# ufal/neuralmonkey

Hardware: NVIDIA H100
Metric: train_target_tokens_per_sec (higher is better)
Workload: dtype f32 storage; tensor-core products in fp16 (vocabulary) / tf32 with fp32 accumulation

## Files before the change

include/nmb200.h:

```cpp
#ifndef NMB200_H
#define NMB200_H

#include <stdint.h>

#ifdef __cplusplus
extern "C" {
#endif

#define NM_ABI_VERSION 1

#define NM_OK 0
#define NM_E_INVALID (-1)
#define NM_E_UNSUPPORTED (-2)
#define NM_E_NO_DEVICE (-3)

#define NM_ACT_NONE 0
#define NM_ACT_TANH 1
#define NM_ACT_RELU 2
#define NM_ACT_SIGMOID 3

#define NM_GEMM_AUTO 0
#define NM_GEMM_SIMT 1
#define NM_GEMM_TC 2

// ... 79 lines not shown
                float* lse, float* xent, int64_t* argmax, int64_t M, int64_t V,
                int64_t ldl, void* stream);
int nm_xent_bwd(const float* logits, const int64_t* targets, const float* weights,
                const float* lse, const float* scale, float* dlogits, int64_t M,
                int64_t V, int64_t ldl, void* stream);
int nm_log_softmax(const float* logits, const float* lse, float* logprobs,
                   int64_t M, int64_t V, int64_t ldl, void* stream);

int64_t nm_logits_xent_scratch(int64_t M, int64_t V);
int nm_logits_xent_fwd(const float* X, int64_t ldx, const float* W, int64_t ldw,
                       int transW, const float* b, int64_t unk_index, const int64_t* targets,
                       const float* weights, float* lse, float* xent,
                       int64_t* argmax, float* part, float* logits_out,
                       int64_t ldl, int64_t M, int64_t V, int64_t K, void* stream);
int nm_logits_xent_bwd(const float* X, int64_t ldx, const float* W, int64_t ldw,
                       int transW, const float* b, int64_t unk_index, const int64_t* targets,
                       const float* weights, const float* lse, const float* scale,
                       float* dlogits, int64_t ldd, int64_t M, int64_t V,
                       int64_t K, void* stream);

int nm_cast_f16(const float* src, int64_t ld_src, void* dst, int64_t ld_dst, int64_t rows,
                int64_t cols, const float* row_scale, int transpose, int extra_ones, void* stream);
int nm_gemm_f16(int64_t M, int64_t N, int64_t K, const void* A16, int64_t lda, const void* B16,
                int64_t ldb, float* C, int64_t ldc, const float* alpha_dev, const float* row_scale,
                float beta, int transposed, void* stream);
int nm_gemm_f16_tn(int64_t M, int64_t N, int64_t K, const void* A16, int64_t lda, const void* B16,
                   int64_t ldb, float* C, int64_t ldc, const float* alpha_dev, float beta, void* stream);
int nm_logits_xent_fwd16(const void* X16, int64_t ldx, const void* WT16, int64_t ldw, const float* b,
                         int64_t unk_index, const int64_t* targets, const float* weights, float* lse,
                         float* xent, int64_t* argmax, float* part, float* logits_out, int64_t ldl,
                         int64_t M, int64_t V, int64_t K, void* stream);
int nm_logits_xent_bwd16(const void* X16, int64_t ldx, const void* WT16, int64_t ldw, const float* b,
                         int64_t unk_index, const int64_t* targets, const float* mask, const float* lse,
                         void* dl16, int64_t ldd, void* dlT16, int64_t lddt, int64_t M, int64_t V,
                         int64_t K, void* stream);

int nm_beam_step(const float* logprobs, const float* logprob_sum,
                 const int32_t* lengths, const uint8_t* finished, float alpha,
                 float* scores, int64_t* word_ids, int32_t* beam_ids,
                 float* logprob_sum_out, int32_t* lengths_out,
                 uint8_t* finished_out, void* scratch, int64_t B, int64_t k,
                 int64_t V, void* stream);
int64_t nm_beam_scratch(int64_t B, int64_t k, int64_t V);
int nm_beam_gather(const void* x, const int32_t* beam_ids, void* out, int64_t B,
                   int64_t k, int64_t row_bytes, void* stream);

int nm_clip_adam_step(float* params, float* grads, float* m, float* v,
                      const int64_t* seg_off, const uint8_t* seg_reg, float* norms,
                      int64_t n, int64_t nseg, float grad_scale,
                      const float* grad_denominator, float lr_t,
                      float beta1, float beta2, float eps, float clip_norm,
                      float l1, float l2, float* l1l2_out,
                      const float* lr_t_dev ,
                      void* stream);

int nm_mha_fwd(const float* q, const float* k, const float* v,
               const float* key_mask, int causal, float* out, float* probs,
               int64_t B, int64_t Tq, int64_t Tk, int64_t heads, int64_t dh,
               void* stream);
int nm_mha_bwd(const float* q, const float* k, const float* v,
               const float* key_mask, int causal, const float* probs,
               const float* dout, float* dq, float* dk, float* dv,
               float* de_work , int64_t B,
               int64_t Tq, int64_t Tk, int64_t heads, int64_t dh, void* stream);
int nm_mha_fwd_drop(const float* q, const float* k, const float* v, const float* key_mask, int causal,
                    const float* drop_mask, float* out, float* probs, int64_t B, int64_t Tq,
                    int64_t Tk, int64_t heads, int64_t dh, void* stream);
int nm_mha_bwd_drop(const float* q, const float* k, const float* v, const float* key_mask, int causal,
// ... 73 lines not shown
```

neuralmonkey_b200/csrc/gemm_tc.cu:

```cuda
#include <cuda.h>
#include <cuda_fp16.h>
#include <stdlib.h>
#include <string.h>

#include "common.cuh"
#include "gemm_tc.h"
#include "tc_ptx.cuh"
#include "wgmma.cuh"

namespace nm {

constexpr int TC_BM = 128;
constexpr int TC_BK = 32;
constexpr int TC_THREADS = 384;
constexpr int TC_EPI_WARPS = 8;
constexpr int TC_A_BYTES = TC_BM * 128;
constexpr int TC_RING_BUDGET = 192 * 1024;

template <int BN>
struct TcCfg {
  static constexpr int B_BYTES = BN * 128;
  static constexpr int STAGE_BYTES = TC_A_BYTES + B_BYTES;
  static constexpr int STAGES = (TC_RING_BUDGET / STAGE_BYTES) > 4 ? 4 : (TC_RING_BUDGET / STAGE_BYTES);
  static constexpr int CT_PITCH = BN + 4;
  static constexpr int RING_BYTES = STAGES * STAGE_BYTES;
  static constexpr int CT_BYTES = TC_BM * CT_PITCH * 4;
  static constexpr int UNION_BYTES = RING_BYTES > CT_BYTES ? RING_BYTES : CT_BYTES;
  static constexpr int SMEM_BYTES = 1024  + UNION_BYTES + 256  +
                                    TC_EPI_WARPS * 4096 ;
  static_assert(SMEM_BYTES <= 227 * 1024, "more shared memory than an sm_90 block may have");
};
struct RowStats {
  float mx, sum, tgt;
  int32_t arg;
};

constexpr float TC_LOG2E = 1.4426950408889634f;

__device__ __forceinline__ float fast_ex2(float x) {
  float y;
  asm("ex2.approx.ftz.f32 %0, %1;" : "=f"(y) : "f"(x));
  return y;
}

__device__ __forceinline__ void load_bias32(const float* __restrict__ bias, int col0, int ncols,
                                            float (&b)[32]) {
  if (bias == nullptr) {
#pragma unroll
    for (int j = 0; j < 32; ++j) b[j] = 0.f;
    return;
  }
  if (ncols == 32 && ((reinterpret_cast<uintptr_t>(bias + col0) & 15) == 0)) {
#pragma unroll
    for (int j = 0; j < 32; j += 4) {
      const float4 v = __ldg(reinterpret_cast<const float4*>(bias + col0 + j));
      b[j] = v.x; b[j + 1] = v.y; b[j + 2] = v.z; b[j + 3] = v.w;
    }
  } else {
#pragma unroll
    for (int j = 0; j < 32; ++j) b[j] = (j < ncols) ? __ldg(bias + col0 + j) : 0.f;
  }
}

__device__ __forceinline__ void store32(float* __restrict__ c, const float (&x)[32], int ncols,
                                        bool vec_ok) {
  if (vec_ok && ncols == 32) {
#pragma unroll
    for (int j = 0; j < 32; j += 4)
      *reinterpret_cast<float4*>(c + j) = make_float4(x[j], x[j + 1], x[j + 2], x[j + 3]);
  } else {
#pragma unroll
    for (int j = 0; j < 32; ++j)
      if (j < ncols) c[j] = x[j];
  }
}

__device__ __forceinline__ void store32_coalesced(float* __restrict__ stage, float* __restrict__ C,
// ... 119 lines not shown
#pragma unroll
    for (int j = 0; j < 8; ++j) {
      float4 v = make_float4(x[4 * j], x[4 * j + 1], x[4 * j + 2], x[4 * j + 3]);
      if (add_bias && e.bias) {
        const float4 b = __ldg(reinterpret_cast<const float4*>(e.bias + col0 + 4 * j));
        v.x += b.x; v.y += b.y; v.z += b.z; v.w += b.w;
      }
      st4[lane * 8 + (j ^ (lane & 7))] = v;
    }
    __syncwarp();
    const int sub = lane >> 3, slot = lane & 7;
    const int64_t row_base = row - lane;
#pragma unroll
    for (int i = 0; i < 8; ++i) {
      const int r = 4 * i + sub;
      const float4 v = st4[r * 8 + (slot ^ (r & 7))];
      const int64_t grow = row_base + r;
      if (grow < M) red_add_v4(e.C + grow * e.ldc + col0 + 4 * slot, v);
    }
    __syncwarp();
    return;
  }
  if (row >= M) return;
  float* c = e.C + row * e.ldc + col0;
#pragma unroll
  for (int j = 0; j < 32; ++j)
    if (j < ncols) {
      float v = x[j];
      if (add_bias && e.bias) v += __ldg(e.bias + col0 + j);
      atomicAdd(c + j, v);
    }
}

template <typename T>
__device__ __forceinline__ void store32_transposed(T* __restrict__ ct, int64_t ldt, int64_t row, int col0,
                                                   int64_t M, int ncols, const float (&x)[32], float beta) {
  if (row >= M) return;
#pragma unroll
  for (int j = 0; j < 32; ++j) {
    if (j < ncols) {
      T* dst = ct + (int64_t)(col0 + j) * ldt + row;
      if constexpr (sizeof(T) == 2) {
        *dst = __float2half_rn(x[j]);
      } else {
        *dst = (beta != 0.f) ? (x[j] + *dst) : x[j];
      }
    }
  }
}

__device__ __forceinline__ void store32_half_coalesced(float* __restrict__ stage, __half* __restrict__ C,
                                                       int64_t ldc, int64_t row_base, int col0, int64_t M,
                                                       const float (&x)[32], int lane) {
  uint4* st4 = reinterpret_cast<uint4*>(stage);
#pragma unroll
  for (int j = 0; j < 4; ++j) {
    __half2 h0 = __floats2half2_rn(x[8 * j], x[8 * j + 1]), h1 = __floats2half2_rn(x[8 * j + 2], x[8 * j + 3]);
    __half2 h2 = __floats2half2_rn(x[8 * j + 4], x[8 * j + 5]), h3 = __floats2half2_rn(x[8 * j + 6], x[8 * j + 7]);
    uint4 v;
    v.x = *reinterpret_cast<uint32_t*>(&h0); v.y = *reinterpret_cast<uint32_t*>(&h1);
    v.z = *reinterpret_cast<uint32_t*>(&h2); v.w = *reinterpret_cast<uint32_t*>(&h3);
    st4[lane * 4 + (j ^ ((lane >> 1) & 3))] = v;
  }
  __syncwarp();
  const int sub = lane >> 2, slot = lane & 3;
#pragma unroll
  for (int i = 0; i < 4; ++i) {
    const int r = 8 * i + sub;
    const uint4 v = st4[r * 4 + (slot ^ ((r >> 1) & 3))];
    const int64_t grow = row_base + r;
    if (grow < M) *reinterpret_cast<uint4*>(C + grow * ldc + col0 + 8 * slot) = v;
  }
  __syncwarp();
}

__device__ __forceinline__ void epilogue_chunk_xent_bwd16(const TcEpilogue& e, const TcExt& ext, float (&x)[32],
                                                          int64_t row, int col0, int64_t M, int N, int target,
                                                          float row_lse2, float row_w,
                                                          float* __restrict__ stage, int lane) {
  if (col0 >= N) return;
  const int ncols = min(32, N - col0);
  float b[32];
  load_bias32(e.bias, col0, ncols, b);
#pragma unroll
  for (int j = 0; j < 32; ++j) x[j] += b[j];
  const int unk_rel = (int)e.unk_index - col0;
  if (unk_rel >= 0 && unk_rel < 32) {
#pragma unroll
    for (int j = 0; j < 32; ++j)
      if (j == unk_rel) x[j] += -1e9f;
  }
#pragma unroll
  for (int j = 0; j < 32; ++j) x[j] = fast_ex2(fmaf(x[j], TC_LOG2E, -row_lse2)) * row_w;
  const int t_rel = target - col0;
  if (t_rel >= 0 && t_rel < ncols) {
#pragma unroll
    for (int j = 0; j < 32; ++j)
      if (j == t_rel) x[j] -= row_w;
  }
  __half* c16 = reinterpret_cast<__half*>(ext.C16);
  const bool vec_ok = ncols == 32 && ((ext.ldc16 & 7) == 0) && ((reinterpret_cast<uintptr_t>(c16) & 15) == 0);
  if (vec_ok) {
    store32_half_coalesced(stage, c16, ext.ldc16, row - lane, col0, M, x, lane);
  } else if (row < M) {
#pragma unroll
    for (int j = 0; j < 32; ++j)
      if (j < ncols) c16[row * ext.ldc16 + col0 + j] = __float2half_rn(x[j]);
  }
  if (ext.C16T)
    store32_transposed(reinterpret_cast<__half*>(ext.C16T), ext.ldc16t, row, col0, M, ncols, x, 0.f);
}

__device__ __forceinline__ void epilogue_chunk_dense16(const TcEpilogue& e, const TcExt& ext, float (&x)[32],
                                                       int64_t row, int col0, int64_t M, int N, float factor,
                                                       bool vec_ok, float* __restrict__ stage, int lane,
                                                       RowStats& st) {
#pragma unroll
  for (int j = 0; j < 32; ++j) x[j] *= factor;
  if (!ext.transposed) {
    epilogue_chunk<TC_EPI_DENSE>(e, x, row, col0, M, N, st, -1, 0.f, 0.f, vec_ok, stage, lane);
    return;
  }
  if (col0 >= N) return;
  const int ncols = min(32, N - col0);
  if (e.bias) {
    float b[32];
    load_bias32(e.bias, col0, ncols, b);
#pragma unroll
    for (int j = 0; j < 32; ++j) x[j] += b[j];
  }
  store32_transposed(e.C, e.ldc, row, col0, M, ncols, x, e.beta);
}

__device__ __forceinline__ void load32_coalesced(float* __restrict__ stage, const float* __restrict__ src,
                                                 int64_t ld, int64_t row_base, int col0, int64_t M,
                                                 float (&x)[32], int lane) {
  float4* st4 = reinterpret_cast<float4*>(stage);
  const int sub = lane >> 3, slot = lane & 7;
#pragma unroll
  for (int i = 0; i < 8; ++i) {
    const int r = 4 * i + sub;
    const int64_t grow = row_base + r;
    float4 v = make_float4(0.f, 0.f, 0.f, 0.f);
// ... 352 lines not shown
typedef CUresult (*EncodeTiledFn)(CUtensorMap*, CUtensorMapDataType, cuuint32_t, void*,
                                  const cuuint64_t*, const cuuint64_t*, const cuuint32_t*,
                                  const cuuint32_t*, CUtensorMapInterleave, CUtensorMapSwizzle,
                                  CUtensorMapL2promotion, CUtensorMapFloatOOBfill);

static EncodeTiledFn get_encode_fn() {
  static EncodeTiledFn fn = nullptr;
  if (!fn) {
    void* p = nullptr;
    cudaDriverEntryPointQueryResult q;
    if (cudaGetDriverEntryPoint("cuTensorMapEncodeTiled", &p, cudaEnableDefault, &q) == cudaSuccess &&
        q == cudaDriverEntryPointSuccess)
      fn = reinterpret_cast<EncodeTiledFn>(p);
  }
  return fn;
}

static int make_map(CUtensorMap* map, const float* base, int64_t rows, int64_t cols, int64_t ld, uint32_t box_rows) {
  EncodeTiledFn fn = get_encode_fn();
  NM_REQUIRE(fn != nullptr, NM_E_NO_DEVICE, "tc_gemm: cuTensorMapEncodeTiled not available");
  const cuuint64_t gdim[2] = {(cuuint64_t)cols, (cuuint64_t)rows};
  const cuuint64_t gstride[1] = {(cuuint64_t)ld * 4};
  const cuuint32_t box[2] = {(cuuint32_t)TC_BK, box_rows};
  const cuuint32_t estr[2] = {1, 1};
  const CUresult r = fn(map, CU_TENSOR_MAP_DATA_TYPE_TFLOAT32, 2, const_cast<float*>(base), gdim, gstride, box, estr,
                        CU_TENSOR_MAP_INTERLEAVE_NONE, CU_TENSOR_MAP_SWIZZLE_128B,
                        CU_TENSOR_MAP_L2_PROMOTION_L2_128B, CU_TENSOR_MAP_FLOAT_OOB_FILL_NONE);
  NM_REQUIRE(r == CUDA_SUCCESS, NM_E_INVALID,
             "tc_gemm: cuTensorMapEncodeTiled failed (%d) rows=%lld cols=%lld ld=%lld", (int)r,
             (long long)rows, (long long)cols, (long long)ld);
  return NM_OK;
}

static int make_map16(CUtensorMap* map, const void* base, int64_t rows, int64_t cols, int64_t ld,
                      uint32_t box_rows) {
  EncodeTiledFn fn = get_encode_fn();
  NM_REQUIRE(fn != nullptr, NM_E_NO_DEVICE, "tc_gemm16: cuTensorMapEncodeTiled not available");
  const cuuint64_t gdim[2] = {(cuuint64_t)cols, (cuuint64_t)rows};
  const cuuint64_t gstride[1] = {(cuuint64_t)ld * 2};
  const cuuint32_t box[2] = {64, box_rows};
  const cuuint32_t estr[2] = {1, 1};
  const CUresult r = fn(map, CU_TENSOR_MAP_DATA_TYPE_FLOAT16, 2, const_cast<void*>(base), gdim, gstride, box,
                        estr, CU_TENSOR_MAP_INTERLEAVE_NONE, CU_TENSOR_MAP_SWIZZLE_128B,
                        CU_TENSOR_MAP_L2_PROMOTION_L2_128B, CU_TENSOR_MAP_FLOAT_OOB_FILL_NONE);
  NM_REQUIRE(r == CUDA_SUCCESS, NM_E_INVALID,
             "tc_gemm16: cuTensorMapEncodeTiled failed (%d) rows=%lld cols=%lld ld=%lld", (int)r,
             (long long)rows, (long long)cols, (long long)ld);
  return NM_OK;
}

static int make_operand(CUtensorMap* map, TcOperand* op, bool mn_major, const void* base, int64_t rows, int64_t cols,
                        int64_t ld, uint32_t box_rows, int esz) {
  memset(map, 0, sizeof(*map));
  *op = TcOperand{base, rows, cols, ld};
  if (mn_major) return NM_OK;
  if (esz == 4) return make_map(map, reinterpret_cast<const float*>(base), rows, cols, ld, box_rows);
  return make_map16(map, base, rows, cols, ld, box_rows);
}

bool tc_gemm_supported(int64_t M, int64_t N, int64_t K, int64_t lda, int64_t ldb, const void* A, const void* B) {
  if (M < 1 || N < 1 || K < 1) return false;
  if ((lda & 3) || (ldb & 3)) return false;
  if (A && (reinterpret_cast<uintptr_t>(A) & 15)) return false;
  if (B && (reinterpret_cast<uintptr_t>(B) & 15)) return false;
  if (M > 0x7fffffffLL || N > 0x7fffffffLL || K > 0x7fffffffLL) return false;
  return true;
}
// ... 233 lines not shown
```

neuralmonkey_b200/csrc/gemm_tc.h:

```cpp
#pragma once
#include <cuda_runtime.h>
#include <stdint.h>

namespace nm {

enum TcEpiMode {
  TC_EPI_DENSE = 0,
  TC_EPI_XENT_FWD = 1,
  TC_EPI_XENT_BWD = 2,
  TC_EPI_XENT_BWD16 = 3,
  TC_EPI_SOFTMAX = 4,
  TC_EPI_DSOFTMAX = 5,
};

constexpr int TC_XENT_BN = 256;

struct TcEpilogue {
  int mode;
  float* C;
  int64_t ldc;
  const float* bias;
  int act;
  float beta;
  int64_t unk_index;
  const int64_t* targets;
  const float* weights;
  const float* lse;
  const float* scale;
  float4* part;
};

struct TcExt {
  void* C16;
  int64_t ldc16;
  void* C16T;
  int64_t ldc16t;
  const float* alpha;
  const float* row_scale;
  int transposed;
};

struct TcBatch {
  int count, inner;
  int a_row_outer, a_row_inner, a_col_inner;
  int b_row_outer, b_row_inner, b_col_inner;
  int64_t c_outer, c_inner;
  float scale;
  int causal;
  const float* key_mask;
  const float* drop;
  float* C2;
  const float* P;
  int m_pad, n_pad;
};

int tc_gemm_batched_launch(int transA, int transB, int64_t M, int64_t N, int64_t K, const float* A, int64_t a_rows,
                           int64_t a_cols, int64_t lda, const float* B, int64_t b_rows, int64_t b_cols,
                           int64_t ldb, const TcEpilogue& epi, const TcBatch& bt, cudaStream_t s);

bool tc_gemm_supported(int64_t M, int64_t N, int64_t K, int64_t lda, int64_t ldb, const void* A, const void* B);

int tc_gemm_launch(int transA, int transB, int64_t M, int64_t N, int64_t K, const float* A,
                   int64_t lda, const float* B, int64_t ldb, const TcEpilogue& epi, cudaStream_t s);

int tc_gemm16_launch(int64_t M, int64_t N, int64_t K, const void* A, int64_t lda, const void* B,
                     int64_t ldb, const TcEpilogue& epi, const TcExt& ext, cudaStream_t s);

int tc_gemm16_mn_launch(int64_t M, int64_t N, int64_t K, const void* A, int64_t lda, const void* B,
                        int64_t ldb, const TcEpilogue& epi, const TcExt& ext, cudaStream_t s);

}
```

neuralmonkey_b200/csrc/tc_ptx.cuh:

```cuda
#pragma once
#include <cuda.h>
#include <cuda_fp16.h>
#include <cuda_runtime.h>
#include <stdint.h>

namespace nm {

__device__ __forceinline__ uint32_t smem_u32(const void* p) {
  return (uint32_t)__cvta_generic_to_shared(p);
}
__device__ __forceinline__ void mbar_init(uint32_t bar, uint32_t count) {
  asm volatile("mbarrier.init.shared::cta.b64 [%0], %1;" ::"r"(bar), "r"(count));
}
__device__ __forceinline__ void mbar_expect_tx(uint32_t bar, uint32_t bytes) {
  asm volatile("mbarrier.arrive.expect_tx.shared::cta.b64 _, [%0], %1;" ::"r"(bar), "r"(bytes)
               : "memory");
}
__device__ __forceinline__ void mbar_arrive(uint32_t bar) {
  asm volatile("mbarrier.arrive.shared::cta.b64 _, [%0];" ::"r"(bar) : "memory");
}
__device__ __forceinline__ void mbar_wait(uint32_t bar, uint32_t parity) {
  asm volatile(
      "{\n\t"
      ".reg .pred p;\n\t"
      "WAIT_LOOP:\n\t"
      "mbarrier.try_wait.parity.shared::cta.b64 p, [%0], %1;\n\t"
      "@p bra WAIT_DONE;\n\t"
      "bra WAIT_LOOP;\n\t"
      "WAIT_DONE:\n\t"
      "}" ::"r"(bar),
      "r"(parity)
      : "memory");
}
__device__ __forceinline__ void tma_load_2d(uint32_t dst, const CUtensorMap* map, uint32_t bar,
                                            int32_t c0, int32_t c1) {
  asm volatile(
      "cp.async.bulk.tensor.2d.shared::cluster.global.mbarrier::complete_tx::bytes"
      " [%0], [%1, {%3, %4}], [%2];" ::"r"(dst),
      "l"(reinterpret_cast<uint64_t>(map)), "r"(bar), "r"(c0), "r"(c1)
      : "memory");
}
__device__ __forceinline__ void mbar_expect_tx_only(uint32_t bar, uint32_t bytes) {
  asm volatile("mbarrier.expect_tx.relaxed.cta.shared::cta.b64 [%0], %1;" ::"r"(bar), "r"(bytes) : "memory");
}
__device__ __forceinline__ uint32_t to_tf32(float x) {
  uint32_t u;
  asm("cvt.rna.tf32.f32 %0, %1;" : "=r"(u) : "f"(x));
  return u;
}

__device__ __forceinline__ void wgmma_fence() { asm volatile("wgmma.fence.sync.aligned;" ::: "memory"); }
__device__ __forceinline__ void wgmma_commit() { asm volatile("wgmma.commit_group.sync.aligned;" ::: "memory"); }
template <int N>
__device__ __forceinline__ void wgmma_wait() {
  asm volatile("wgmma.wait_group.sync.aligned %0;" ::"n"(N) : "memory");
}
template <int R>
__device__ __forceinline__ void wgmma_fence_operands(float (&d)[R]) {
#pragma unroll
  for (int i = 0; i < R; ++i) asm volatile("" : "+f"(d[i])::"memory");
}

__device__ __forceinline__ uint64_t gmma_desc_sw128(uint32_t addr) {
  return (uint64_t)((addr & 0x3FFFFu) >> 4) | ((uint64_t)1 << 16) | ((uint64_t)(1024 >> 4) << 32) |
         ((uint64_t)1 << 62);
}

__device__ __forceinline__ uint64_t gmma_desc_sw128_mn(uint32_t addr) {
  return (uint64_t)((addr & 0x3FFFFu) >> 4) | ((uint64_t)(8192 >> 4) << 16) | ((uint64_t)(1024 >> 4) << 32) |
         ((uint64_t)1 << 62);
}

}
```

neuralmonkey_b200/csrc/xent16.cu:

```cuda
#include <cuda_fp16.h>

#include "common.cuh"
#include "gemm_tc.h"

namespace nm {

__global__ void cast_f16_kernel(const float* __restrict__ src, int64_t ld_src, __half* __restrict__ dst,
                                int64_t ld_dst, int64_t rows, int64_t cols,
                                const float* __restrict__ row_scale, int extra_ones) {
  const int64_t total = rows * ld_dst;
  for (int64_t i = blockIdx.x * (int64_t)blockDim.x + threadIdx.x; i < total;
       i += (int64_t)gridDim.x * blockDim.x) {
    const int64_t r = i / ld_dst, c = i - r * ld_dst;
    float v = 0.f;
    const float sc = row_scale ? row_scale[r] : 1.f;
    if (c < cols) v = src[r * ld_src + c] * sc;
    else if (c < cols + extra_ones) v = sc;
    dst[i] = __float2half_rn(v);
  }
}

__global__ void cast_transpose_f16_kernel(const float* __restrict__ src, int64_t ld_src,
                                          __half* __restrict__ dst, int64_t ld_dst, int64_t rows,
                                          int64_t cols, const float* __restrict__ row_scale,
                                          int extra_ones) {
  __shared__ float tile[32][33];
  const int64_t r0 = blockIdx.x * 32LL, c0 = blockIdx.y * 32LL;
  for (int i = threadIdx.y; i < 32; i += blockDim.y) {
    const int64_t r = r0 + i, c = c0 + threadIdx.x;
    float v = 0.f;
    if (r < rows) {
      const float sc = row_scale ? row_scale[r] : 1.f;
      if (c < cols) v = src[r * ld_src + c] * sc;
      else if (c < cols + extra_ones) v = sc;
    }
    tile[i][threadIdx.x] = v;
  }
  __syncthreads();
  for (int i = threadIdx.y; i < 32; i += blockDim.y) {
    const int64_t c = c0 + i, r = r0 + threadIdx.x;
    if (c < cols + extra_ones && r < ld_dst) dst[c * ld_dst + r] = __float2half_rn(tile[threadIdx.x][i]);
  }
}

}

using namespace nm;

extern "C" {

int nm_cast_f16(const float* src, int64_t ld_src, void* dst, int64_t ld_dst, int64_t rows, int64_t cols,
                const float* row_scale, int transpose, int extra_ones, void* stream) {
  NM_REQUIRE(src && dst && rows > 0 && cols > 0 && ld_src >= cols, NM_E_INVALID, "nm_cast_f16: bad arguments");
  cudaStream_t s = (cudaStream_t)stream;
  if (!transpose) {
    NM_REQUIRE(extra_ones >= 0 && ld_dst >= cols + extra_ones, NM_E_INVALID, "nm_cast_f16: bad destination pitch");
    const int64_t total = rows * ld_dst;
    const int64_t blocks = ceil_div(total, 256 * 4);
    const int64_t cap = (int64_t)sm_count() * 16;
    cast_f16_kernel<<<(unsigned)(blocks < cap ? blocks : cap), 256, 0, s>>>(
        src, ld_src, reinterpret_cast<__half*>(dst), ld_dst, rows, cols, row_scale, extra_ones);
  } else {
    NM_REQUIRE(ld_dst >= rows && extra_ones >= 0, NM_E_INVALID, "nm_cast_f16: bad destination pitch");
    const dim3 grid((unsigned)ceil_div(ld_dst, 32), (unsigned)ceil_div(cols + extra_ones, 32));
    cast_transpose_f16_kernel<<<grid, dim3(32, 8), 0, s>>>(src, ld_src, reinterpret_cast<__half*>(dst), ld_dst,
                                                          rows, cols, row_scale, extra_ones);
  }
  NM_LAUNCH_CHECK("nm_cast_f16");
  return NM_OK;
}

int nm_gemm_f16(int64_t M, int64_t N, int64_t K, const void* A16, int64_t lda, const void* B16, int64_t ldb,
                float* C, int64_t ldc, const float* alpha_dev, const float* row_scale, float beta,
                int transposed, void* stream) {
  NM_REQUIRE(A16 && B16 && C, NM_E_INVALID, "nm_gemm_f16: null pointer");
// ... 2 lines not shown
  TcEpilogue epi{};
  epi.mode = TC_EPI_DENSE;
  epi.C = C;
  epi.ldc = ldc;
  epi.act = NM_ACT_NONE;
  epi.beta = beta;
  epi.unk_index = -1;
  TcExt ext{};
  ext.alpha = alpha_dev;
  ext.row_scale = row_scale;
  ext.transposed = transposed;
  return tc_gemm16_launch(M, N, K, A16, lda, B16, ldb, epi, ext, (cudaStream_t)stream);
}

int nm_gemm_f16_tn(int64_t M, int64_t N, int64_t K, const void* A16, int64_t lda, const void* B16, int64_t ldb,
                   float* C, int64_t ldc, const float* alpha_dev, float beta, void* stream) {
  NM_REQUIRE(A16 && B16 && C, NM_E_INVALID, "nm_gemm_f16_tn: null pointer");
  NM_REQUIRE(beta == 0.f || beta == 1.f, NM_E_INVALID, "nm_gemm_f16_tn: beta must be 0 or 1");
  NM_REQUIRE(lda >= M && ldb >= N && ldc >= N, NM_E_INVALID, "nm_gemm_f16_tn: bad pitches");
  TcEpilogue epi{};
  epi.mode = TC_EPI_DENSE;
  epi.C = C;
  epi.ldc = ldc;
  epi.act = NM_ACT_NONE;
  epi.beta = beta;
  epi.unk_index = -1;
  TcExt ext{};
  ext.alpha = alpha_dev;
  return tc_gemm16_mn_launch(M, N, K, A16, lda, B16, ldb, epi, ext, (cudaStream_t)stream);
}

int nm_logits_xent_bwd16(const void* X16, int64_t ldx, const void* WT16, int64_t ldw, const float* b,
                         int64_t unk_index, const int64_t* targets, const float* mask, const float* lse,
                         void* dl16, int64_t ldd, void* dlT16, int64_t lddt, int64_t M, int64_t V, int64_t K,
                         void* stream) {
  NM_REQUIRE(X16 && WT16 && targets && lse && dl16, NM_E_INVALID, "nm_logits_xent_bwd16: null pointer");
  NM_REQUIRE(M > 0 && V > 0 && K > 0 && ldx >= K && ldw >= K && ldd >= V && (!dlT16 || lddt >= M),
             NM_E_INVALID, "nm_logits_xent_bwd16: bad sizes");
  TcEpilogue epi{};
  epi.mode = TC_EPI_XENT_BWD16;
  epi.bias = b;
  epi.unk_index = unk_index;
  epi.targets = targets;
  epi.weights = mask;
  epi.lse = lse;
  TcExt ext{};
  ext.C16 = dl16;
  ext.ldc16 = ldd;
  ext.C16T = dlT16;
  ext.ldc16t = lddt;
  return tc_gemm16_launch(M, V, K, X16, ldx, WT16, ldw, epi, ext, (cudaStream_t)stream);
}

}
```

neuralmonkey_b200/csrc/xent_tc.cu:

```cuda
#include "common.cuh"
#include "gemm_tc.h"

namespace nm {

__global__ void xent_combine_kernel(const float4* __restrict__ part, int64_t M, int64_t tiles_n,
                                    const int64_t* __restrict__ targets,
                                    const float* __restrict__ weights, float* __restrict__ lse,
                                    float* __restrict__ xent, int64_t* __restrict__ argmax) {
  const int lane = threadIdx.x & 31;
  const int64_t row = blockIdx.x * (int64_t)(blockDim.x >> 5) + (threadIdx.x >> 5);
  if (row >= M) return;
  float mx = -INFINITY, tgt = -INFINITY;
  int32_t arg = 0x7fffffff;
  for (int64_t t = lane; t < tiles_n; t += 32) {
    const float4 p = part[row * tiles_n + t];
    const int32_t a = __float_as_int(p.z);
    if (p.x > mx || (p.x == mx && a < arg)) { mx = p.x; arg = a; }
    tgt = fmaxf(tgt, p.w);
  }
#pragma unroll
  for (int o = 16; o > 0; o >>= 1) {
    const float omx = __shfl_xor_sync(0xffffffffu, mx, o);
    const int32_t oarg = __shfl_xor_sync(0xffffffffu, arg, o);
    if (omx > mx || (omx == mx && oarg < arg)) { mx = omx; arg = oarg; }
// ... 55 lines not shown
  return NM_OK;
}

int nm_logits_xent_bwd(const float* X, int64_t ldx, const float* W, int64_t ldw, int transW,
                       const float* b, int64_t unk_index, const int64_t* targets, const float* weights,
                       const float* lse, const float* scale, float* dlogits, int64_t ldd, int64_t M,
                       int64_t V, int64_t K, void* stream) {
  NM_REQUIRE(X && W && targets && lse && scale && dlogits, NM_E_INVALID,
             "nm_logits_xent_bwd: null pointer");
  NM_REQUIRE(M > 0 && V > 0 && K > 0 && ldx >= K && ldw >= (transW ? K : V) && ldd >= V, NM_E_INVALID,
             "nm_logits_xent_bwd: bad sizes");
  NM_REQUIRE(tc_gemm_supported(M, V, K, ldx, ldw, X, W), NM_E_UNSUPPORTED,
             "nm_logits_xent_bwd: operands not TMA-addressable (use nm_gemm + nm_xent_bwd)");
  TcEpilogue epi{};
  epi.mode = TC_EPI_XENT_BWD;
  epi.C = dlogits;
  epi.ldc = ldd;
  epi.bias = b;
  epi.unk_index = unk_index;
  epi.targets = targets;
  epi.weights = weights;
  epi.lse = lse;
  epi.scale = scale;
  return tc_gemm_launch(0, transW, M, V, K, X, ldx, W, ldw, epi, (cudaStream_t)stream);
}

int nm_logits_xent_fwd16(const void* X16, int64_t ldx, const void* WT16, int64_t ldw, const float* b,
                         int64_t unk_index, const int64_t* targets, const float* weights, float* lse,
                         float* xent, int64_t* argmax, float* part, float* logits_out, int64_t ldl,
                         int64_t M, int64_t V, int64_t K, void* stream) {
  NM_REQUIRE(X16 && WT16 && lse && part, NM_E_INVALID, "nm_logits_xent_fwd16: null pointer");
  NM_REQUIRE(M > 0 && V > 0 && K > 0 && ldx >= K && ldw >= K, NM_E_INVALID, "nm_logits_xent_fwd16: bad sizes");
  NM_REQUIRE(!logits_out || ldl >= V, NM_E_INVALID, "nm_logits_xent_fwd16: ldl < V");
  cudaStream_t s = (cudaStream_t)stream;
  TcEpilogue epi{};
  epi.mode = TC_EPI_XENT_FWD;
  epi.C = logits_out;
  epi.ldc = ldl;
  epi.bias = b;
  epi.unk_index = unk_index;
  epi.targets = targets;
  epi.part = reinterpret_cast<float4*>(part);
  const int rc = tc_gemm16_launch(M, V, K, X16, ldx, WT16, ldw, epi, TcExt{}, s);
  if (rc) return rc;
  const int64_t tiles_n = 2 * ceil_div(V, TC_XENT_BN);
  xent_combine_kernel<<<(unsigned)ceil_div(M, 8), 256, 0, s>>>(reinterpret_cast<const float4*>(part), M,
                                                              tiles_n, targets, weights, lse, xent, argmax);
  NM_LAUNCH_CHECK("nm_logits_xent_fwd16(combine)");
  return NM_OK;
}

}
```

neuralmonkey_b200/ops.py:

```python
import os
from typing import Optional, Tuple

import torch

from neuralmonkey_b200 import lib
from neuralmonkey_b200.lib import call, ptr

_GEMM_BACKEND = lib.GEMM_AUTO


def set_gemm_backend(name: str) -> None:
    global _GEMM_BACKEND
    _GEMM_BACKEND = {"auto": lib.GEMM_AUTO, "simt": lib.GEMM_SIMT, "tc": lib.GEMM_TC}[name]
    call("nm_gru_set_mode", 1 if name == "simt" else 0)


def gemm_backend() -> int:
    return _GEMM_BACKEND


def _f32(t: torch.Tensor) -> torch.Tensor:
    if t.dtype != torch.float32:
        raise TypeError("expected float32, got {}".format(t.dtype))
    return t
# ... 644 lines not shown
        w2, ldw = _rows(w)
        x16 = torch.empty(m, kpad, device=dev, dtype=torch.float16)
        call("nm_cast_f16", ptr(x2), ldx, ptr(x16), kpad, m, k, None, 0, 0, lib.stream())
        wt16 = torch.empty(v, kpad, device=dev, dtype=torch.float16)
        call("nm_cast_f16", ptr(w2), ldw, ptr(wt16), kpad, k, v, None, 1, 0, lib.stream())
        lse = torch.empty(m, device=dev, dtype=torch.float32)
        xent = torch.empty(m, device=dev, dtype=torch.float32)
        argmax = torch.empty(m, device=dev, dtype=torch.int64)
        logits = torch.empty(m, v, device=dev, dtype=torch.float32) if keep_logits else None
        part = torch.empty(lib.load().nm_logits_xent_scratch(m, v), device=dev, dtype=torch.float32)
        call("nm_logits_xent_fwd16", ptr(x16), kpad, ptr(wt16), kpad, ptr(b), unk_index, ptr(targets),
             ptr(weights), ptr(lse), ptr(xent), ptr(argmax), ptr(part), ptr(logits), v, m, v, k,
             lib.stream())
        ctx.save_for_backward(x2, w2, b, targets, weights, lse, x16, wt16)
        ctx.cfg = (unk_index, x.shape)
        ctx.sinks = (_sink(w), _sink(b) if b is not None else None)
        ctx.mark_non_differentiable(lse, argmax)
        if keep_logits:
            ctx.mark_non_differentiable(logits)
        return xent, lse, argmax, logits

    @staticmethod
    def backward(ctx, dxent, _dlse, _dargmax, _dlogits):
        x2, w2, b, targets, weights, lse, x16, wt16 = ctx.saved_tensors
        unk_index, in_shape = ctx.cfg
        m, k = x2.shape
        v = w2.size(1)
        dev = x2.device
        kpad, vpad = _pad8(k), _pad8(v)
        _, ldx = _rows(x2)
        _, ldw = _rows(w2)
        dl16 = torch.empty(m, vpad, device=dev, dtype=torch.float16)
        call("nm_logits_xent_bwd16", ptr(x16), kpad, ptr(wt16), kpad, ptr(b), unk_index, ptr(targets),
             ptr(weights), ptr(lse), ptr(dl16), vpad, None, 0, m, v, k, lib.stream())
        upstream = dxent.reshape(-1).to(torch.float32).contiguous()
        dx = None
        if ctx.needs_input_grad[0]:
            w16 = torch.empty(k, vpad, device=dev, dtype=torch.float16)
            call("nm_cast_f16", ptr(w2), ldw, ptr(w16), vpad, k, v, None, 0, 0, lib.stream())
            dx = torch.empty(m, k, device=dev, dtype=torch.float32)
            call("nm_gemm_f16", m, k, v, ptr(dl16), vpad, ptr(w16), vpad, ptr(dx), k, None,
                 ptr(upstream), 0.0, 0, lib.stream())
            dx = dx.view(in_shape)
        w_sink, _b_sink = ctx.sinks
        smax = upstream.abs().amax().clamp_min(1e-30).reshape(1)
        k1pad = _pad8(k + 1)
        xs16 = torch.empty(m, k1pad, device=dev, dtype=torch.float16)
        call("nm_cast_f16", ptr(x2), ldx, ptr(xs16), k1pad, m, k, ptr(upstream / smax), 0, 1, lib.stream())
        sink_aug = torch.as_strided(w_sink, (k + 1, v), (v, 1))
        _off_the_chain(lambda: call("nm_gemm_f16_tn", k + 1, v, m, ptr(xs16), k1pad, ptr(dl16), vpad, ptr(sink_aug),
                                    v, ptr(smax), 1.0, lib.stream()), xs16, dl16, smax, sink_aug)
        return dx, None, None, None, None, None, None


class _LogitsXent(torch.autograd.Function):

    @staticmethod
    def forward(ctx, x, w, b, targets, weights, unk_index, trans_w, keep_logits):
        x2 = x.reshape(-1, x.shape[-1])
        x2, ldx = _rows(x2)
        m, k = x2.shape
        v = w.size(0) if trans_w else w.size(1)
        dev = x.device
        targets = targets.reshape(-1).contiguous()
        weights = weights.reshape(-1).contiguous()
        lse = torch.empty(m, device=dev, dtype=torch.float32)
        xent = torch.empty(m, device=dev, dtype=torch.float32)
# ... 339 lines not shown
```

Measured before the change: 1.054 million.

## Add dedicated persistent fp16 fused logits-xent kernel keeping vocab tile resident across K

Adds a warp-specialized persistent WGMMA kernel for the fused vocabulary projection plus cross-entropy forward and backward when K is at most 320. The whole K extent of a vocabulary tile stays resident in shared memory and is reused across consecutive M tiles, while two consumer warpgroups ping-pong so one runs its epilogue while the other runs MMAs. The backward pass writes dlogits through stmatrix staging with evict-first stores. The unused transposed fp16 output path is removed. The aim is less reloading of the weight tile and better overlap of the epilogue, at the cost of a second specialized code path and a hard K limit.

```diff
diff --git a/include/nmb200.h b/include/nmb200.h
--- a/include/nmb200.h
+++ b/include/nmb200.h
@@ -135,8 +135,7 @@
                          int64_t M, int64_t V, int64_t K, void* stream);
 int nm_logits_xent_bwd16(const void* X16, int64_t ldx, const void* WT16, int64_t ldw, const float* b,
                          int64_t unk_index, const int64_t* targets, const float* mask, const float* lse,
-                         void* dl16, int64_t ldd, void* dlT16, int64_t lddt, int64_t M, int64_t V,
-                         int64_t K, void* stream);
+                         void* dl16, int64_t ldd, int64_t M, int64_t V, int64_t K, void* stream);
 
 int nm_beam_step(const float* logprobs, const float* logprob_sum,
                  const int32_t* lengths, const uint8_t* finished, float alpha,
diff --git a/neuralmonkey_b200/csrc/gemm_tc.cu b/neuralmonkey_b200/csrc/gemm_tc.cu
--- a/neuralmonkey_b200/csrc/gemm_tc.cu
+++ b/neuralmonkey_b200/csrc/gemm_tc.cu
@@ -35,14 +35,6 @@
   int32_t arg;
 };
 
-constexpr float TC_LOG2E = 1.4426950408889634f;
-
-__device__ __forceinline__ float fast_ex2(float x) {
-  float y;
-  asm("ex2.approx.ftz.f32 %0, %1;" : "=f"(y) : "f"(x));
-  return y;
-}
-
 __device__ __forceinline__ void load_bias32(const float* __restrict__ bias, int col0, int ncols,
                                             float (&b)[32]) {
   if (bias == nullptr) {
@@ -228,19 +220,14 @@
     }
 }
 
-template <typename T>
-__device__ __forceinline__ void store32_transposed(T* __restrict__ ct, int64_t ldt, int64_t row, int col0,
+__device__ __forceinline__ void store32_transposed(float* __restrict__ ct, int64_t ldt, int64_t row, int col0,
                                                    int64_t M, int ncols, const float (&x)[32], float beta) {
   if (row >= M) return;
 #pragma unroll
   for (int j = 0; j < 32; ++j) {
     if (j < ncols) {
-      T* dst = ct + (int64_t)(col0 + j) * ldt + row;
-      if constexpr (sizeof(T) == 2) {
-        *dst = __float2half_rn(x[j]);
-      } else {
-        *dst = (beta != 0.f) ? (x[j] + *dst) : x[j];
-      }
+      float* dst = ct + (int64_t)(col0 + j) * ldt + row;
+      *dst = (beta != 0.f) ? (x[j] + *dst) : x[j];
     }
   }
 }
@@ -303,8 +290,6 @@
     for (int j = 0; j < 32; ++j)
       if (j < ncols) c16[row * ext.ldc16 + col0 + j] = __float2half_rn(x[j]);
   }
-  if (ext.C16T)
-    store32_transposed(reinterpret_cast<__half*>(ext.C16T), ext.ldc16t, row, col0, M, ncols, x, 0.f);
 }
 
 __device__ __forceinline__ void epilogue_chunk_dense16(const TcEpilogue& e, const TcExt& ext, float (&x)[32],
@@ -723,7 +708,7 @@
   return NM_OK;
 }
 
-static int make_map16(CUtensorMap* map, const void* base, int64_t rows, int64_t cols, int64_t ld,
+int make_map16(CUtensorMap* map, const void* base, int64_t rows, int64_t cols, int64_t ld,
                       uint32_t box_rows) {
   EncodeTiledFn fn = get_encode_fn();
   NM_REQUIRE(fn != nullptr, NM_E_NO_DEVICE, "tc_gemm16: cuTensorMapEncodeTiled not available");
diff --git a/neuralmonkey_b200/csrc/gemm_tc.h b/neuralmonkey_b200/csrc/gemm_tc.h
--- a/neuralmonkey_b200/csrc/gemm_tc.h
+++ b/neuralmonkey_b200/csrc/gemm_tc.h
@@ -1,4 +1,5 @@
 #pragma once
+#include <cuda.h>
 #include <cuda_runtime.h>
 #include <stdint.h>
 
@@ -33,8 +34,6 @@
 struct TcExt {
   void* C16;
   int64_t ldc16;
-  void* C16T;
-  int64_t ldc16t;
   const float* alpha;
   const float* row_scale;
   int transposed;
@@ -58,6 +57,14 @@
                            int64_t a_cols, int64_t lda, const float* B, int64_t b_rows, int64_t b_cols,
                            int64_t ldb, const TcEpilogue& epi, const TcBatch& bt, cudaStream_t s);
 
+int make_map16(CUtensorMap* map, const void* base, int64_t rows, int64_t cols, int64_t ld, uint32_t box_rows);
+
+constexpr int64_t XENT16_MAX_K = 320;
+int xent16_launch(bool bwd, const void* X16, int64_t ldx, const void* WT16, int64_t ldw, const float* b,
+                  int64_t unk_index, const int64_t* targets, const float* mask, const float* lse, float4* part,
+                  float* logits_out, int64_t ldl, void* dl16, int64_t ldd, int64_t M, int64_t V, int64_t K,
+                  cudaStream_t s);
+
 bool tc_gemm_supported(int64_t M, int64_t N, int64_t K, int64_t lda, int64_t ldb, const void* A, const void* B);
 
 int tc_gemm_launch(int transA, int transB, int64_t M, int64_t N, int64_t K, const float* A,
diff --git a/neuralmonkey_b200/csrc/tc_ptx.cuh b/neuralmonkey_b200/csrc/tc_ptx.cuh
--- a/neuralmonkey_b200/csrc/tc_ptx.cuh
+++ b/neuralmonkey_b200/csrc/tc_ptx.cuh
@@ -43,6 +43,14 @@
 __device__ __forceinline__ void mbar_expect_tx_only(uint32_t bar, uint32_t bytes) {
   asm volatile("mbarrier.expect_tx.relaxed.cta.shared::cta.b64 [%0], %1;" ::"r"(bar), "r"(bytes) : "memory");
 }
+constexpr float TC_LOG2E = 1.4426950408889634f;
+
+__device__ __forceinline__ float fast_ex2(float x) {
+  float y;
+  asm("ex2.approx.ftz.f32 %0, %1;" : "=f"(y) : "f"(x));
+  return y;
+}
+
 __device__ __forceinline__ uint32_t to_tf32(float x) {
   uint32_t u;
   asm("cvt.rna.tf32.f32 %0, %1;" : "=r"(u) : "f"(x));
diff --git a/neuralmonkey_b200/csrc/xent16.cu b/neuralmonkey_b200/csrc/xent16.cu
--- a/neuralmonkey_b200/csrc/xent16.cu
+++ b/neuralmonkey_b200/csrc/xent16.cu
@@ -2,6 +2,8 @@
 
 #include "common.cuh"
 #include "gemm_tc.h"
+#include "tc_ptx.cuh"
+#include "wgmma.cuh"
 
 namespace nm {
 
@@ -41,6 +43,337 @@
     const int64_t c = c0 + i, r = r0 + threadIdx.x;
     if (c < cols + extra_ones && r < ld_dst) dst[c * ld_dst + r] = __float2half_rn(tile[threadIdx.x][i]);
   }
+}
+
+constexpr int X16_BM = 64;
+constexpr int X16_BN = TC_XENT_BN;
+constexpr int X16_A_BYTES = X16_BM * 128;
+constexpr int X16_B_BYTES = X16_BN * 128;
+constexpr int X16_B_SLOTS = XENT16_MAX_K / 64;
+constexpr int X16_STAGE_WARP = 16 * 128 * 2;
+constexpr int X16_THREADS = 384;
+
+template <bool BWD>
+struct X16Cfg {
+  static constexpr int A_STAGES = BWD ? 4 : 8;
+  static constexpr int A_OFF = X16_B_SLOTS * X16_B_BYTES;
+  static constexpr int ST_OFF = A_OFF + A_STAGES * X16_A_BYTES;
+  static constexpr int BAR_OFF = ST_OFF + (BWD ? 8 * X16_STAGE_WARP : 0);
+  static constexpr int SMEM_BYTES = 1024  + BAR_OFF + 256 ;
+  static_assert(SMEM_BYTES <= 227 * 1024, "more shared memory than an sm_90 block may have");
+  static_assert((2 * A_STAGES + 2 * X16_B_SLOTS) * 8 <= 256, "barrier area");
+};
+
+struct X16Args {
+  const float* bias;
+  int64_t unk;
+  const int64_t* targets;
+  const float* mask;
+  const float* lse;
+  float4* part;
+  float* logits;
+  int64_t ldl;
+  __half* dl16;
+  int64_t ldd;
+  int M, V, K;
+};
+
+__device__ __forceinline__ void named_sync(int id) { asm volatile("bar.sync %0, 256;" ::"r"(id) : "memory"); }
+__device__ __forceinline__ void named_arrive(int id) { asm volatile("bar.arrive %0, 256;" ::"r"(id) : "memory"); }
+
+__device__ __forceinline__ uint32_t pack_half2(float lo, float hi) {
+  __half2 h = __floats2half2_rn(lo, hi);
+  return *reinterpret_cast<uint32_t*>(&h);
+}
+
+__device__ __forceinline__ void merge_stats(float& mx, float& sum, int& arg, float& tgt, float omx, float osum,
+                                            int oarg, float otgt) {
+  const float nm = fmaxf(mx, omx);
+  if (nm != -INFINITY) sum = sum * fast_ex2((mx - nm) * TC_LOG2E) + osum * fast_ex2((omx - nm) * TC_LOG2E);
+  if (omx > mx || (omx == mx && oarg < arg)) arg = oarg;
+  mx = nm;
+  tgt = fmaxf(tgt, otgt);
+}
+
+template <bool BWD>
+__global__ void __launch_bounds__(X16_THREADS, 1)
+xent16_kernel(const __grid_constant__ CUtensorMap map_x, const __grid_constant__ CUtensorMap map_w, X16Args p) {
+  using Cfg = X16Cfg<BWD>;
+  constexpr int AST = Cfg::A_STAGES;
+  extern __shared__ uint8_t smem_raw[];
+  uint8_t* smem = smem_raw + ((1024u - (smem_u32(smem_raw) & 1023u)) & 1023u);
+  const uint32_t sbase = smem_u32(smem);
+  const uint32_t bars = sbase + Cfg::BAR_OFF;
+  auto full_a = [&](int s) { return bars + 8u * s; };
+  auto empty_a = [&](int s) { return bars + 8u * (AST + s); };
+  auto full_b = [&](int s) { return bars + 8u * (2 * AST + s); };
+  auto empty_b = [&](int s) { return bars + 8u * (2 * AST + X16_B_SLOTS + s); };
+
+  const int tiles_m = (p.M + X16_BM - 1) / X16_BM;
+  const int units = tiles_m * ((p.V + X16_BN - 1) / X16_BN);
+  const int first = (int)((int64_t)blockIdx.x * units / gridDim.x);
+  const int count = (int)((int64_t)(blockIdx.x + 1) * units / gridDim.x) - first;
+  const int KB = (p.K + 63) / 64;
+
+  if (threadIdx.x == 0) {
+    asm volatile("prefetch.tensormap [%0];" ::"l"(reinterpret_cast<uint64_t>(&map_x)) : "memory");
+    asm volatile("prefetch.tensormap [%0];" ::"l"(reinterpret_cast<uint64_t>(&map_w)) : "memory");
+    for (int s = 0; s < AST; ++s) {
+      mbar_init(full_a(s), 1);
+      mbar_init(empty_a(s), 4);
+    }
+    for (int s = 0; s < X16_B_SLOTS; ++s) {
+      mbar_init(full_b(s), 1);
+      mbar_init(empty_b(s), 4);
+    }
+    asm volatile("fence.mbarrier_init.release.cluster;" ::: "memory");
+    asm volatile("fence.proxy.async.shared::cta;" ::: "memory");
+  }
+  __syncthreads();
+  const int warp = threadIdx.x >> 5, lane = threadIdx.x & 31;
+
+  if (warp < 4) {
+    asm volatile("setmaxnreg.dec.sync.aligned.u32 40;" ::: "memory");
+    if (threadIdx.x != 0) return;
+    int loads = 0, prev_tn = -1;
+    for (int j = 0; j < count; ++j) {
+      const int u = first + j, tm = u % tiles_m, tn = u / tiles_m;
+      const bool reload = tn != prev_tn;
+      loads += reload;
+      prev_tn = tn;
+      for (int kb = 0; kb < KB; ++kb) {
+        const int ia = j * KB + kb, sa = ia % AST;
+        mbar_wait(empty_a(sa), ((ia / AST) & 1) ^ 1u);
+        mbar_expect_tx(full_a(sa), X16_A_BYTES);
+        tma_load_2d(sbase + Cfg::A_OFF + sa * X16_A_BYTES, &map_x, full_a(sa), kb * 64, tm * X16_BM);
+        if (reload) {
+          mbar_wait(empty_b(kb), ((loads - 1) & 1) ^ 1u);
+          mbar_expect_tx(full_b(kb), X16_B_BYTES);
+          tma_load_2d(sbase + kb * X16_B_BYTES, &map_w, full_b(kb), kb * 64, tn * X16_BN);
+        }
+      }
+    }
+    return;
+  }
+
+  asm volatile("setmaxnreg.inc.sync.aligned.u32 232;" ::: "memory");
+  const int c = (warp >> 2) - 1;
+  const int w = warp & 3, q = lane & 3;
+  uint64_t evict_first = 0;
+  if (BWD) asm volatile("createpolicy.fractional.L2::evict_first.b64 %0, 1.0;" : "=l"(evict_first));
+  if (c == 1) named_arrive(1);
+  float acc[128];
+  int loads = 0, prev_tn = -1;
+  for (int j = 0; j < count; ++j) {
+    const int u = first + j, tm = u % tiles_m, tn = u / tiles_m;
+    loads += tn != prev_tn;
+    prev_tn = tn;
+    if ((j & 1) != c) continue;
+    const bool last_use = j + 1 == count || (u + 1) / tiles_m != tn;
+
+    named_sync(1 + c);
+#pragma unroll
+    for (int i = 0; i < 128; ++i) acc[i] = 0.f;
+    for (int kb = 0; kb < KB; ++kb) {
+      const int ia = j * KB + kb, sa = ia % AST;
+      mbar_wait(full_a(sa), (ia / AST) & 1);
+      mbar_wait(full_b(kb), (loads - 1) & 1);
+      const uint32_t a_addr = sbase + Cfg::A_OFF + sa * X16_A_BYTES, b_addr = sbase + kb * X16_B_BYTES;
+      wgmma_fence();
+#pragma unroll
+      for (int k = 0; k < 4; ++k)
+        Wgmma<256, 2>::mma(acc, gmma_desc_sw128(a_addr + k * 32), gmma_desc_sw128(b_addr + k * 32));
+      wgmma_commit();
+      wgmma_wait<1>();
+      wgmma_fence_operands(acc);
+      if (kb > 0 && lane == 0) mbar_arrive(empty_a((ia - 1) % AST));
+    }
+    wgmma_wait<0>();
+    wgmma_fence_operands(acc);
+    if (lane == 0) {
+      mbar_arrive(empty_a((j * KB + KB - 1) % AST));
+      if (last_use)
+        for (int kb = 0; kb < KB; ++kb) mbar_arrive(empty_b(kb));
+    }
+    if (j + 1 < count) named_arrive(2 - c);
+
+    const int r0 = tm * X16_BM + 16 * w + (lane >> 2);
+    const int n0 = tn * X16_BN, cb = n0 + 2 * q;
+    const int V = p.V;
+#pragma unroll
+    for (int i = 0; i < 32; ++i) {
+#pragma unroll
+      for (int e = 0; e < 2; ++e) {
+        const int col = cb + 8 * i + e;
+        const float b = (p.bias != nullptr && col < V) ? __ldg(p.bias + col) : 0.f;
+        acc[4 * i + e] += b;
+        acc[4 * i + 2 + e] += b;
+      }
+    }
+    const int unk_rel = (int)(p.unk - cb);
+    if (p.unk >= 0 && unk_rel >= 0 && unk_rel < X16_BN && (unk_rel & 6) == 0) {
+#pragma unroll
+      for (int i = 0; i < 32; ++i)
+#pragma unroll
+        for (int e = 0; e < 2; ++e)
+          if (8 * i + e == unk_rel) {
+            acc[4 * i + e] += -1e9f;
+            acc[4 * i + 2 + e] += -1e9f;
+          }
+    }
+#pragma unroll
+    for (int h = 0; h < 2; ++h) {
+      const int row = r0 + 8 * h;
+      const bool row_ok = row < p.M;
+      const int target = (row_ok && p.targets) ? (int)p.targets[row] : -1;
+      const int t_rel = target - cb;
+      const bool has_t = target >= 0 && t_rel >= 0 && t_rel < X16_BN && (t_rel & 6) == 0;
+      if constexpr (!BWD) {
+        if (p.logits && row_ok) {
+          float* lrow = p.logits + (int64_t)row * p.ldl + cb;
+          const int ncols = V - cb;
+#pragma unroll
+          for (int i = 0; i < 32; ++i)
+#pragma unroll
+            for (int e = 0; e < 2; ++e)
+              if (8 * i + e < ncols) lrow[8 * i + e] = acc[4 * i + 2 * h + e];
+        }
+        if (n0 + X16_BN > V) {
+#pragma unroll
+          for (int i = 0; i < 32; ++i)
+#pragma unroll
+            for (int e = 0; e < 2; ++e)
+              if (cb + 8 * i + e >= V) acc[4 * i + 2 * h + e] = -INFINITY;
+        }
+        float mx = -INFINITY;
+        int arg = 0x7fffffff;
+#pragma unroll
+        for (int i = 0; i < 32; ++i)
+#pragma unroll
+          for (int e = 0; e < 2; ++e)
+            if (acc[4 * i + 2 * h + e] > mx) {
+              mx = acc[4 * i + 2 * h + e];
+              arg = cb + 8 * i + e;
+            }
+        const float m2 = mx == -INFINITY ? 0.f : mx * TC_LOG2E;
+        float s[4] = {0.f, 0.f, 0.f, 0.f};
+#pragma unroll
+        for (int i = 0; i < 32; ++i)
+#pragma unroll
+          for (int e = 0; e < 2; ++e)
+            s[(2 * i + e) & 3] += fast_ex2(fmaf(acc[4 * i + 2 * h + e], TC_LOG2E, -m2));
+        float sum = (s[0] + s[1]) + (s[2] + s[3]);
+        float tgt = -INFINITY;
+        if (has_t) {
+#pragma unroll
+          for (int i = 0; i < 32; ++i)
+#pragma unroll
+            for (int e = 0; e < 2; ++e)
+              if (8 * i + e == t_rel) tgt = acc[4 * i + 2 * h + e];
+        }
+        merge_stats(mx, sum, arg, tgt, __shfl_xor_sync(0xffffffffu, mx, 1), __shfl_xor_sync(0xffffffffu, sum, 1),
+                    __shfl_xor_sync(0xffffffffu, arg, 1), __shfl_xor_sync(0xffffffffu, tgt, 1));
+        if (row_ok && (q & 1) == h) {
+          const int tiles_n2 = 2 * ((V + X16_BN - 1) / X16_BN);
+          p.part[(int64_t)row * tiles_n2 + 2 * tn + (q >> 1)] = make_float4(mx, sum, __int_as_float(arg), tgt);
+        }
+      } else {
+        const float lse2 = row_ok ? p.lse[row] * TC_LOG2E : 0.f;
+        const float wt = row_ok ? (p.mask ? p.mask[row] : 1.f) : 0.f;
+#pragma unroll
+        for (int i = 0; i < 32; ++i)
+#pragma unroll
+          for (int e = 0; e < 2; ++e)
+            acc[4 * i + 2 * h + e] = fast_ex2(fmaf(acc[4 * i + 2 * h + e], TC_LOG2E, -lse2)) * wt;
+        if (has_t) {
+#pragma unroll
+          for (int i = 0; i < 32; ++i)
+#pragma unroll
+            for (int e = 0; e < 2; ++e)
+              if (8 * i + e == t_rel) acc[4 * i + 2 * h + e] -= wt;
+        }
+      }
+    }
+    if constexpr (BWD) {
+      uint8_t* stage = smem + Cfg::ST_OFF + (warp - 4) * X16_STAGE_WARP;
+      const uint32_t stage_u = smem_u32(stage);
+      const int srow_w = (lane & 7) + ((lane >> 3) & 1) * 8;
+#pragma unroll
+      for (int half = 0; half < 2; ++half) {
+#pragma unroll
+        for (int jj = 0; jj < 16; jj += 2) {
+          const int i = 16 * half + jj;
+          const int chunk = jj + (lane >> 4);
+          const uint32_t addr = stage_u + srow_w * 256 + ((chunk ^ (srow_w & 7)) << 4);
+          asm volatile("stmatrix.sync.aligned.m8n8.x4.shared.b16 [%0], {%1, %2, %3, %4};" ::"r"(addr),
+                       "r"(pack_half2(acc[4 * i], acc[4 * i + 1])), "r"(pack_half2(acc[4 * i + 2], acc[4 * i + 3])),
+                       "r"(pack_half2(acc[4 * i + 4], acc[4 * i + 5])), "r"(pack_half2(acc[4 * i + 6], acc[4 * i + 7]))
+                       : "memory");
+        }
+        __syncwarp();
+#pragma unroll
+        for (int it = 0; it < 8; ++it) {
+          const int idx = it * 32 + lane, srow = idx >> 4, ch = idx & 15;
+          const uint4 v = *reinterpret_cast<const uint4*>(stage + srow * 256 + ((ch ^ (srow & 7)) << 4));
+          const int grow = tm * X16_BM + 16 * w + srow;
+          const int gcol = n0 + 128 * half + 8 * ch;
+          if (grow < p.M && gcol < V) {
+            __half* dst = p.dl16 + (int64_t)grow * p.ldd + gcol;
+            if (gcol + 8 <= V) {
+              asm volatile("st.global.L2::cache_hint.v4.b32 [%0], {%1, %2, %3, %4}, %5;" ::"l"(dst), "r"(v.x),
+                           "r"(v.y), "r"(v.z), "r"(v.w), "l"(evict_first)
+                           : "memory");
+            } else {
+              const uint32_t wv[4] = {v.x, v.y, v.z, v.w};
+#pragma unroll
+              for (int e = 0; e < 8; ++e)
+                if (gcol + e < V) dst[e] = __ushort_as_half((unsigned short)(wv[e >> 1] >> (16 * (e & 1))));
+            }
+          }
+        }
+        __syncwarp();
+      }
+    }
+  }
+}
+
+template <bool BWD>
+static int launch_xent16(const CUtensorMap& mx, const CUtensorMap& mw, const X16Args& a, int grid, cudaStream_t s,
+                         const char* name) {
+  auto kern = xent16_kernel<BWD>;
+  static bool attr_done = false;
+  if (!attr_done) {
+    NM_CUDA_TRY(cudaFuncSetAttribute(kern, cudaFuncAttributeMaxDynamicSharedMemorySize, X16Cfg<BWD>::SMEM_BYTES));
+    attr_done = true;
+  }
+  kern<<<grid, X16_THREADS, X16Cfg<BWD>::SMEM_BYTES, s>>>(mx, mw, a);
+  NM_LAUNCH_CHECK(name);
+  return NM_OK;
+}
+
+int xent16_launch(bool bwd, const void* X16, int64_t ldx, const void* WT16, int64_t ldw, const float* b,
+                  int64_t unk_index, const int64_t* targets, const float* mask, const float* lse, float4* part,
+                  float* logits_out, int64_t ldl, void* dl16, int64_t ldd, int64_t M, int64_t V, int64_t K,
+                  cudaStream_t s) {
+  const char* name = bwd ? "nm_logits_xent_bwd16" : "nm_logits_xent_fwd16";
+  NM_REQUIRE(ceil_div(M, X16_BM) * ceil_div(V, X16_BN) <= 0x7fffffffLL && M * 2 * ceil_div(V, X16_BN) <= 0x7fffffffLL &&
+                 K <= XENT16_MAX_K,
+             NM_E_INVALID, "%s: shape %lld x %lld x %lld too large", name, (long long)M, (long long)V, (long long)K);
+  NM_REQUIRE((ldx & 7) == 0 && (ldw & 7) == 0 && (reinterpret_cast<uintptr_t>(X16) & 15) == 0 &&
+                 (reinterpret_cast<uintptr_t>(WT16) & 15) == 0,
+             NM_E_INVALID, "%s: fp16 operands need 16-byte aligned bases and row pitches", name);
+  NM_REQUIRE(!bwd || ((ldd & 7) == 0 && (reinterpret_cast<uintptr_t>(dl16) & 15) == 0), NM_E_INVALID,
+             "%s: dl16 needs a 16-byte aligned base and row pitch", name);
+  CUtensorMap mx, mw;
+  int rc = make_map16(&mx, X16, M, K, ldx, X16_BM);
+  if (rc) return rc;
+  rc = make_map16(&mw, WT16, V, K, ldw, X16_BN);
+  if (rc) return rc;
+  X16Args a{b, unk_index, targets, mask, lse, part, logits_out, ldl, reinterpret_cast<__half*>(dl16), ldd,
+            (int)M, (int)V, (int)K};
+  const int64_t units = ceil_div(M, X16_BM) * ceil_div(V, X16_BN);
+  const int grid = (int)(units < sm_count() ? units : sm_count());
+  return bwd ? launch_xent16<true>(mx, mw, a, grid, s, name) : launch_xent16<false>(mx, mw, a, grid, s, name);
 }
 
 }
@@ -109,11 +442,13 @@
 
 int nm_logits_xent_bwd16(const void* X16, int64_t ldx, const void* WT16, int64_t ldw, const float* b,
                          int64_t unk_index, const int64_t* targets, const float* mask, const float* lse,
-                         void* dl16, int64_t ldd, void* dlT16, int64_t lddt, int64_t M, int64_t V, int64_t K,
-                         void* stream) {
+                         void* dl16, int64_t ldd, int64_t M, int64_t V, int64_t K, void* stream) {
   NM_REQUIRE(X16 && WT16 && targets && lse && dl16, NM_E_INVALID, "nm_logits_xent_bwd16: null pointer");
-  NM_REQUIRE(M > 0 && V > 0 && K > 0 && ldx >= K && ldw >= K && ldd >= V && (!dlT16 || lddt >= M),
-             NM_E_INVALID, "nm_logits_xent_bwd16: bad sizes");
+  NM_REQUIRE(M > 0 && V > 0 && K > 0 && ldx >= K && ldw >= K && ldd >= V, NM_E_INVALID,
+             "nm_logits_xent_bwd16: bad sizes");
+  if (K <= XENT16_MAX_K)
+    return xent16_launch(true, X16, ldx, WT16, ldw, b, unk_index, targets, mask, lse, nullptr, nullptr, 0, dl16,
+                         ldd, M, V, K, (cudaStream_t)stream);
   TcEpilogue epi{};
   epi.mode = TC_EPI_XENT_BWD16;
   epi.bias = b;
@@ -124,8 +459,6 @@
   TcExt ext{};
   ext.C16 = dl16;
   ext.ldc16 = ldd;
-  ext.C16T = dlT16;
-  ext.ldc16t = lddt;
   return tc_gemm16_launch(M, V, K, X16, ldx, WT16, ldw, epi, ext, (cudaStream_t)stream);
 }
 
diff --git a/neuralmonkey_b200/csrc/xent_tc.cu b/neuralmonkey_b200/csrc/xent_tc.cu
--- a/neuralmonkey_b200/csrc/xent_tc.cu
+++ b/neuralmonkey_b200/csrc/xent_tc.cu
@@ -111,16 +111,24 @@
   NM_REQUIRE(X16 && WT16 && lse && part, NM_E_INVALID, "nm_logits_xent_fwd16: null pointer");
   NM_REQUIRE(M > 0 && V > 0 && K > 0 && ldx >= K && ldw >= K, NM_E_INVALID, "nm_logits_xent_fwd16: bad sizes");
   NM_REQUIRE(!logits_out || ldl >= V, NM_E_INVALID, "nm_logits_xent_fwd16: ldl < V");
+  NM_REQUIRE((reinterpret_cast<uintptr_t>(part) & 15) == 0, NM_E_INVALID,
+             "nm_logits_xent_fwd16: part must be 16-byte aligned");
   cudaStream_t s = (cudaStream_t)stream;
-  TcEpilogue epi{};
-  epi.mode = TC_EPI_XENT_FWD;
-  epi.C = logits_out;
-  epi.ldc = ldl;
-  epi.bias = b;
-  epi.unk_index = unk_index;
-  epi.targets = targets;
-  epi.part = reinterpret_cast<float4*>(part);
-  const int rc = tc_gemm16_launch(M, V, K, X16, ldx, WT16, ldw, epi, TcExt{}, s);
+  int rc;
+  if (K <= XENT16_MAX_K) {
+    rc = xent16_launch(false, X16, ldx, WT16, ldw, b, unk_index, targets, nullptr, nullptr,
+                       reinterpret_cast<float4*>(part), logits_out, ldl, nullptr, 0, M, V, K, s);
+  } else {
+    TcEpilogue epi{};
+    epi.mode = TC_EPI_XENT_FWD;
+    epi.C = logits_out;
+    epi.ldc = ldl;
+    epi.bias = b;
+    epi.unk_index = unk_index;
+    epi.targets = targets;
+    epi.part = reinterpret_cast<float4*>(part);
+    rc = tc_gemm16_launch(M, V, K, X16, ldx, WT16, ldw, epi, TcExt{}, s);
+  }
   if (rc) return rc;
   const int64_t tiles_n = 2 * ceil_div(V, TC_XENT_BN);
   xent_combine_kernel<<<(unsigned)ceil_div(M, 8), 256, 0, s>>>(reinterpret_cast<const float4*>(part), M,
diff --git a/neuralmonkey_b200/ops.py b/neuralmonkey_b200/ops.py
--- a/neuralmonkey_b200/ops.py
+++ b/neuralmonkey_b200/ops.py
@@ -700,7 +700,7 @@
         _, ldw = _rows(w2)
         dl16 = torch.empty(m, vpad, device=dev, dtype=torch.float16)
         call("nm_logits_xent_bwd16", ptr(x16), kpad, ptr(wt16), kpad, ptr(b), unk_index, ptr(targets),
-             ptr(weights), ptr(lse), ptr(dl16), vpad, None, 0, m, v, k, lib.stream())
+             ptr(weights), ptr(lse), ptr(dl16), vpad, m, v, k, lib.stream())
         upstream = dxent.reshape(-1).to(torch.float32).contiguous()
         dx = None
         if ctx.needs_input_grad[0]:
```

Measured after the change: 1.121 million (median of 6 runs). 6.3% higher.
